# NTT123/vietTTS

Measured on NVIDIA H100. Metric: audio_samples_per_sec, higher is better.
Workload: dtype f32 (bf16x3 split products on wgmma tensor cores, fp32 accumulate/storage)

## Files before the change

### viettts_b200/csrc/hifigan.cu

```cuda
#include "vtts_internal.cuh"

using namespace hgpk;

namespace {

__global__ void repack_ups_kernel(const float* __restrict__ w, float* __restrict__ out, int u, int K, int Cin, int Cout, int a) {
  const size_t total = (size_t)u * 2 * Cin * Cout;
  for (size_t idx = blockIdx.x * (size_t)blockDim.x + threadIdx.x; idx < total; idx += (size_t)gridDim.x * blockDim.x) {
    int o = idx % Cout;
    int i = (idx / Cout) % Cin;
    int q = (idx / ((size_t)Cout * Cin)) % 2;
    int r = idx / ((size_t)Cout * Cin * 2);
    int j0 = ((a - r) % u + u) % u;
    int j = j0 + q * u;
    out[idx] = w[((size_t)j * Cout + o) * Cin + i];
  }
}

__global__ void __launch_bounds__(256) conv_post_kernel(const float* __restrict__ a0, const float* __restrict__ a1,
                                                        const float* __restrict__ a2, const float* __restrict__ w,
                                                        const float* __restrict__ bias, const int* __restrict__ len,
                                                        int len_mul, int R, float* __restrict__ wav) {
  constexpr int C = 32, KW = 7, TT = 256, ST = 33;
  __shared__ float xs[(TT + KW - 1) * ST];
// ... 54 lines not shown

void carve(Arena& ar, int B, int T, HgBufs& hb) {
  const size_t frames = (size_t)B * T;
  hb.P0 = ar.take<float>(frames * 512);
  const size_t big = frames * 8192;
  for (int p = 0; p < 2; ++p)
    for (int j = 0; j < 3; ++j) hb.A[p][j] = ar.take<float>(big);
  hb.X = ar.take<float>(big);
  for (int j = 0; j < 3; ++j) hb.Tb[j] = ar.take<float>(big);
  for (int j = 0; j < 3; ++j) hb.Bb[j] = ar.take<float>(big);
}

}

size_t vtts_hifigan_ws_bytes(int B, int T) {
  Arena ar(nullptr, 0, true);
  HgBufs hb;
  carve(ar, B, T, hb);
  return ar.off + 256;
}

int vtts_hifigan_prepare(vtts_ctx* ctx) {
  ModelWeights& m = ctx->hg;
  std::vector<size_t> dn;
  for (int i = 0, C = vc::HG_C0; i < 4; ++i, C /= 2) dn.push_back((size_t)vc::hg_rate(i) * 2 * C * (C / 2));
  int rc = vtts_alloc_tensors(ctx, dn, &m.derived, m.d);
  if (rc) return rc;
  std::vector<PackSpec> pk(2 * PK_COUNT);
  for (int i = 0, C = vc::HG_C0; i < 4; ++i, C /= 2) {
    const int u = vc::hg_rate(i), K = vc::hg_upk(i);
    repack_ups_kernel<<<256, 256>>>(m.t[hgi::UPS_W(i)], m.d[i], u, K, C, C / 2, (K + u - 2 + 1) / 2);
    VTTS_CUDA(cudaGetLastError());
    for (int r = 0; r < u; ++r) pk[PK_UPS(i, r)] = {m.d[i] + (size_t)r * 2 * C * (C / 2), 2, C, C / 2};
  }
  for (int n = 0; n < 12; ++n)
    for (int which = 0; which < 2; ++which)
      for (int j = 0; j < 3; ++j) {
        const int ch = 256 >> (n / 3);
        pk[PK_RB(n, which, j)] = {m.t[hgi::RB_W(n, which, j)], vc::hg_rbk(n % 3), ch, ch};
      }
  pk[PK_PRE] = {m.t[hgi::PRE_W], 7, vc::MEL, vc::HG_C0};
  for (int e = 0; e < PK_COUNT; ++e) {
    pk[PK_COUNT + e] = pk[e];
    pk[PK_COUNT + e].f16 = true;
  }
  VTTS_CUDA(cudaDeviceSynchronize());
  rc = vtts_pack_convs(ctx, m, pk);
  if (rc) return rc;
  VTTS_CUDA(cudaDeviceSynchronize());
  return VTTS_OK;
}


namespace {

int hg_scale(int i) {
// ... 28 lines not shown
}

int hg_ups(vtts_ctx* ctx, int i, const float* const* x, float* out, const int32_t* n_frames, int B, int T, cudaStream_t st) {
  const ModelWeights& M = ctx->hg;
  auto& W = M.t;
  const bool tc = ctx->precision != VTTS_PRECISION_FP32;
  const int f16 = ctx->precision == VTTS_PRECISION_FP16;
  const int pk = f16 ? PK_COUNT : 0;
  const int C = vc::HG_C0 >> i, scale_in = hg_scale(i), rows_in = T * scale_in;
  const int u = vc::hg_rate(i), K = vc::hg_upk(i), Co = C / 2;
  const int a = (K + u - 2 + 1) / 2;
  ConvLaunch L;
  memset(&L, 0, sizeof(L));
  L.B = B; L.len = n_frames; L.len_mul = scale_in;
  L.nprob = u; L.Cin = C; L.Cout = Co;
  L.T_rows = rows_in; L.rows_out = rows_in * u;
  L.pre_mode = (i == 0) ? 1 : 2; L.pre_slope = 0.1f; L.post_act = 0;
  for (int r = 0; r < u; ++r) {
    int j0 = ((a - r) % u + u) % u;
    int e = (r + j0 - a) / u;
    ConvProb p;
    memset(&p, 0, sizeof(p));
    if (i == 0) { p.x0 = x[0]; } else { p.x0 = x[0]; p.x1 = x[1]; p.x2 = x[2]; }
    p.w = M.d[i] + (size_t)r * 2 * C * Co;
    p.bias = W[hgi::UPS_B(i)];
    p.out = out;
    p.k = 2; p.dil = 1; p.in_off = e; p.out_stride = u; p.out_off = r;
    L.p[r] = p;
  }
  if (!tc) return vtts_launch_conv(ctx, L, st);
  const int nph = Co == 256 ? 1 : (Co == 128 ? 4 : 2);
  TcLaunch TL;
  memset(&TL, 0, sizeof(TL));
  TL.nprob = u / nph; TL.nphase = nph; TL.Cin = C; TL.N = Co; TL.in_ld = C; TL.out_ld = Co;
  TL.B = B; TL.T_rows = rows_in; TL.rows_out = rows_in * u; TL.len = n_frames; TL.len_mul = scale_in;
  TL.pre_mode = L.pre_mode; TL.pre_slope = 0.1f; TL.f16 = f16;
  for (int g = 0; g < u / nph; ++g) {
    const ConvProb& c0 = L.p[g * nph];
    TcProb q;
    memset(&q, 0, sizeof(q));
    q.x0 = c0.x0; q.x1 = c0.x1; q.x2 = c0.x2; q.bias = c0.bias; q.out = c0.out;
    q.k = 2; q.dil = 1; q.out_stride = u;
    q.wpk = M.tiles(pk + PK_UPS(i, g * nph))[0]; q.in_off = c0.in_off; q.out_off = g * nph;
    for (int ph = 0; ph < nph; ++ph) {
      const int r = g * nph + ph;
      q.wpk_ph[ph] = M.tiles(pk + PK_UPS(i, r))[0];
      q.in_off_ph[ph] = L.p[r].in_off;
      q.out_off_ph[ph] = r;
    }
    TL.p[g] = q;
  }
  return vtts_launch_tc_conv(ctx, TL, st);
}

int hg_resblock(vtts_ctx* ctx, int i, int m, const float* const* src, float* const* dst, float* const* tmp, const int32_t* n_frames,
                int B, int T, cudaStream_t st) {
  const ModelWeights& M = ctx->hg;
  auto& W = M.t;
  const bool tc = ctx->precision != VTTS_PRECISION_FP32;
  const int f16 = ctx->precision == VTTS_PRECISION_FP16;
  const int pk = f16 ? PK_COUNT : 0;
  const int Co = vc::HG_C0 >> (i + 1), scale = hg_scale(i + 1), rows = T * scale;
  const int d = vc::hg_dil(m);
  if (tc && ctx->fuse_pairs && Co <= 64) {
    TcPairLaunch PL;
    memset(&PL, 0, sizeof(PL));
    PL.nprob = 3; PL.N = Co; PL.B = B; PL.T_rows = rows; PL.len = n_frames; PL.len_mul = scale; PL.slope = 0.1f; PL.f16 = f16;
    for (int j = 0; j < 3; ++j) {
      const int kk = vc::hg_rbk(j), n = i * 3 + j;
      PL.p[j] = TcPairProb{src[j], M.tiles(pk + PK_RB(n, 0, m))[0], M.tiles(pk + PK_RB(n, 1, m))[0], W[hgi::RB_B(n, 0, m)], W[hgi::RB_B(n, 1, m)],
                           dst[j], kk, d};
    }
    return vtts_launch_tc_pair(ctx, PL, st);
// ... 146 lines not shown
```

### viettts_b200/csrc/tc_conv.cu

```cuda
#include <cuda_bf16.h>

#include <algorithm>

#include "tc_common.cuh"
#include "vtts_internal.cuh"

namespace {

using namespace tcx;

constexpr int NCWG = 2;
constexpr int NCONS = NCWG * 128;
constexpr int PROD_WARP = NCONS / 32;
constexpr int NCONV = 96;
constexpr int NTHREADS = NCONS + 32 + NCONV;
constexpr int NA = 4;
constexpr int HALO = 64;
constexpr int PAIR_OVERLAP = 16;
constexpr int NQ = 2;
constexpr int NREADERS = (NCONS + NCONV) / 32;

template <int N, int MW, int PAIRF, bool STAGED = false>
struct TcCfg {
  static constexpr int R = 64 * MW * NCWG;
  static constexpr int R_OUT = R - PAIR_OVERLAP;
  static constexpr int RA = R + HALO;
  static constexpr int A_STAGE = RA * 64;
  static constexpr int W_STAGE = N * 64;
  static constexpr int NW = N == 256 ? 4 : 8;
  static constexpr int NCH2 = PAIRF ? N / 16 : 0;
  static constexpr int EPI_NC = N < 128 ? N : 128;
  static constexpr int EPI_LD = EPI_NC + 8;
  static constexpr int EPI_WG = 64 * EPI_LD + N;
  static constexpr int EPI_STAGE = STAGED ? NCWG * EPI_WG * 4 : 0;
  static constexpr int SMEM_BYTES =
      NA * A_STAGE + NW * W_STAGE + NCH2 * A_STAGE + EPI_STAGE + (2 * NA + 2 * NW + 2 * NQ) * 8 + NQ * 4 + 1024;
  static_assert(SMEM_BYTES <= 227 * 1024, "shared memory of one CTA");
};

struct Ring {
  uint32_t s = 0, p = 0;
  template <int NS>
  __device__ __forceinline__ void next() { if (++s == NS) { s = 0; p ^= 1; } }
};

struct Tile {
  int pi, b, tt, ph;
};
__device__ __forceinline__ Tile decode_tile(int t, int nph, int nprob, int tiles_per_row) {
  Tile d;
  d.ph = t % nph; t /= nph;
  d.pi = t % nprob; t /= nprob;
  d.tt = t % tiles_per_row;
  d.b = t / tiles_per_row;
  return d;
}

__device__ __forceinline__ int take_ticket(int* sched, int ntiles) {
  const int t = (int)gridDim.x + atomicAdd(&sched[0], 1);
  if (t < ntiles) return t;
  __threadfence();
  if (atomicAdd(&sched[1], 1) == (int)gridDim.x - 1) {
    atomicExch(&sched[0], 0);
    atomicExch(&sched[1], 0);
  }
  return -1;
}

struct TileQueue {
  int* id;
  uint64_t* full;
  uint64_t* empty;
  Ring r;
  __device__ __forceinline__ void put(int t, int* err, long long& acc) {
// ... 160 lines not shown
  asm volatile("cp.async.cg.shared.global [%0], [%1], 16;" ::"r"(smem_u32(smem_dst)), "l"(gsrc) : "memory");
}
__device__ __forceinline__ void cp_async_commit() { asm volatile("cp.async.commit_group;" ::: "memory"); }
__device__ __forceinline__ void cp_async_wait_all() { asm volatile("cp.async.wait_all;" ::: "memory"); }

__device__ __forceinline__ void init_barriers(uint64_t* bars, int nw) {
  uint64_t* a_full = bars;
  uint64_t* a_empty = bars + NA;
  uint64_t* w_full = bars + 2 * NA;
  uint64_t* w_empty = bars + 2 * NA + nw;
  uint64_t* q_full = bars + 2 * NA + 2 * nw;
  uint64_t* q_empty = q_full + NQ;
  for (int i = 0; i < NA; ++i) { mbar_init(&a_full[i], NCONV); mbar_init(&a_empty[i], NCONS / 32); }
  for (int i = 0; i < nw; ++i) { mbar_init(&w_full[i], 1); mbar_init(&w_empty[i], NCONS / 32); }
  for (int i = 0; i < NQ; ++i) { mbar_init(&q_full[i], 1); mbar_init(&q_empty[i], NREADERS); }
  asm volatile("fence.mbarrier_init.release.cluster;" ::: "memory");
}

__device__ __forceinline__ TileQueue tile_queue(uint64_t* bars, int nw) {
  uint64_t* q_full = bars + 2 * NA + 2 * nw;
  return TileQueue{reinterpret_cast<int*>(q_full + 2 * NQ), q_full, q_full + NQ, Ring{}};
}

#define PRODUCER_TILES                                                                     \
  TileQueue q = tile_queue(bars, NW);                                                      \
  long long w_q = 0;                                                                       \
  int t_next = blockIdx.x;                                                                 \
  q.put(t_next, L.err, w_q);                                                               \
  auto next_tile = [&]() {                                                                 \
    const int t = t_next;                                                                  \
    if (t >= 0) { t_next = take_ticket(L.sched, L.ntiles); q.put(t_next, L.err, w_q); }    \
    return t;                                                                              \
  };
#define READER_TILES                                                                       \
  TileQueue q = tile_queue(bars, NW);                                                      \
  long long w_q = 0;                                                                       \
  auto next_tile = [&]() { return q.get(L.err, w_q); };

template <int N, int EPI, int MW, bool F16>
__global__ void __launch_bounds__(NTHREADS, 1) tc_conv_kernel(const __grid_constant__ TcLaunch L) {
  using Cfg = TcCfg<N, MW, 0, EPI == 0>;
  constexpr int R = Cfg::R, RA = Cfg::RA, NW = Cfg::NW;
  extern __shared__ uint8_t smem_raw[];
  uint8_t* smem = (uint8_t*)(((uintptr_t)smem_raw + 1023) & ~(uintptr_t)1023);
  uint8_t* a_st = smem;
  uint8_t* w_st = smem + NA * Cfg::A_STAGE;
  float* epi_st = reinterpret_cast<float*>(smem_raw + (w_st + NW * Cfg::W_STAGE - smem_raw));
  uint64_t* bars = reinterpret_cast<uint64_t*>(w_st + NW * Cfg::W_STAGE + Cfg::EPI_STAGE);
  uint64_t* a_full = bars;
  uint64_t* a_empty = bars + NA;
  uint64_t* w_full = bars + 2 * NA;
  uint64_t* w_empty = bars + 2 * NA + NW;

  const int tid = threadIdx.x;
  const int warp = __shfl_sync(0xffffffffu, tid >> 5, 0);
  if (tid == 0) init_barriers(bars, NW);
  __syncthreads();

  const int nch = L.Cin / 16;
  const int nph = L.nphase > 1 ? L.nphase : 1;

  constexpr bool ROW_BOUNDS = EPI == 0;
#define TILE_LOOP_BEGIN                                                           \
  for (int tile; (tile = next_tile()) >= 0;) {                                    \
    const Tile td = decode_tile(tile, nph, L.nprob, L.tiles_per_row);              \
    const int ph = td.ph, b = td.b;                                                 \
    const int tau0 = td.tt * R;                                                    \
    const TcProb& P = L.p[td.pi];                                                  \
    int valid = L.T_rows, in_lo = 0, out_hi = 0;                                  \
    if (ROW_BOUNDS && P.rb) {                                                     \
      in_lo = P.rb[3 * b]; valid = P.rb[3 * b + 1]; out_hi = P.rb[3 * b + 2];     \
      if (tau0 * P.out_stride + P.out_off_ph[ph] >= out_hi) continue;             \
    } else {                                                                      \
      if (L.len) {                                                                \
        const int v = L.len[b] * L.len_mul;                                       \
        valid = v < valid ? v : valid;                                            \
      }                                                                           \
      if (tau0 >= valid) continue;                                                \
    }
#define TILE_LOOP_END }

  if (warp == PROD_WARP) {
    if ((tid & 31) == 0) {
      Ring rw;
      long long w_e = 0;
      PRODUCER_TILES
      TILE_LOOP_BEGIN
        (void)b; (void)tau0; (void)in_lo; (void)valid; (void)out_hi;
        produce_weights<N, NW, F16>(w_st, w_full, w_empty, rw, P.wpk_ph[ph], nch, P.k, L.err, w_e);
      TILE_LOOP_END
      if (L.dbg) L.dbg[(size_t)blockIdx.x * 16 + 4] = w_e;
    }
  } else if (warp > PROD_WARP) {
    const int ct = tid - NCONS - 32;
    Ring ra;
    long long w_ae = 0;
    READER_TILES
    TILE_LOOP_BEGIN
      const int k = P.k, dil = P.dil;
      const size_t in_base = (size_t)b * L.T_rows * L.in_ld;
      const float* x1 = L.pre_mode == 2 ? P.x1 + in_base : nullptr;
      const float* x2 = L.pre_mode == 2 ? P.x2 + in_base : nullptr;
      for (int c = 0; c < nch; ++c) {
        mbar_wait_t(&a_empty[ra.s], ra.p ^ 1, L.err, 5, w_ae);
        convert_chunk<RA, F16>(a_st + ra.s * Cfg::A_STAGE, ct, P.x0 + in_base, x1, x2, L.in_ld, c, tau0 + P.in_off_ph[ph], R + (k - 1) * dil,
                          in_lo, valid, L.pre_mode, L.pre_slope);
        fence_proxy_async();
        mbar_arrive(&a_full[ra.s]);
        ra.next<NA>();
      }
      (void)out_hi;
    TILE_LOOP_END
    if (L.dbg && ct == 0) L.dbg[(size_t)blockIdx.x * 16 + 5] = w_ae;
  } else {
    const int wg = warp >> 2, lane = tid & 31;
    float acc[MW][N / 2];
    Ring ra, rw;
    long long w_a = 0, w_w = 0, t_epi = 0;
    const long long t_begin = clock64();
    const int n_valid = (EPI && L.n_valid > 0) ? L.n_valid : N;
    const int post_act = EPI ? L.post_act : 0;
    constexpr int EPI_NC = Cfg::EPI_NC, EPI_LD = Cfg::EPI_LD, RPS = 128 / (EPI_NC / 4), NQ4 = 64 / RPS;
    float* stg = epi_st + wg * Cfg::EPI_WG;
    float* stg_bias = stg + 64 * EPI_LD;
    const int fr = (warp & 3) * 16 + (lane >> 2), fc = 2 * (lane & 3);
    const int dr = (tid & 127) / (EPI_NC / 4), dq = (tid & 127) % (EPI_NC / 4);
    READER_TILES
    TILE_LOOP_BEGIN
      const size_t out_base = (size_t)b * L.rows_out * L.out_ld;
      const int ostride = P.out_stride, ooff = P.out_off_ph[ph];
      auto row_ok = [&](int tau) { return (ROW_BOUNDS && P.rb) ? tau * ostride + ooff < out_hi : tau < valid; };
      auto fetch_pass = [&](int mt, int nh) {
        if (P.resid) {
          const int blk = tau0 + (wg * MW + mt) * 64;
#pragma unroll
          for (int i = 0; i < NQ4; ++i) {
            const int row = i * RPS + dr, tau = blk + row;
            if (row_ok(tau))
              cp_async16(stg + row * EPI_LD + dq * 4, P.resid + out_base + ((tau * ostride + ooff) * L.out_ld + nh * EPI_NC + dq * 4));
          }
        }
        cp_async_commit();
      };
      auto wait_pass = [&]() {
        cp_async_wait_all();
        named_bar(2 + wg, 128);
      };
      if constexpr (EPI == 0) {
        if ((tid & 127) < N / 4) cp_async16(stg_bias + (tid & 127) * 4, P.bias + (tid & 127) * 4);
        fetch_pass(0, 0);
      }
      consume<N, MW, RA, NW, true, false, F16>(acc, wg, smem_u32(a_st), a_full, a_empty, ra, smem_u32(w_st), w_full, w_empty, rw, nch, P.k,
                                               P.dil, L.err, w_a, w_w);
      const long long t_epi0 = clock64();
      if constexpr (EPI == 0) {
        wait_pass();
#pragma unroll
        for (int mt = 0; mt < MW; ++mt) {
          if (!row_ok(tau0 + (wg * MW + mt) * 64)) break;
#pragma unroll
          for (int nh = 0; nh < N / EPI_NC; ++nh) {
            if (mt + nh > 0 && P.resid) {
              fetch_pass(mt, nh);
              wait_pass();
            }
#pragma unroll
            for (int jn = 0; jn < EPI_NC / 8; ++jn) {
              const int col = jn * 8 + fc, e = (nh * (EPI_NC / 8) + jn) * 4;
              const float2 bi = *reinterpret_cast<const float2*>(stg_bias + nh * EPI_NC + col);
#pragma unroll
              for (int h = 0; h < 2; ++h) {
                float2* s = reinterpret_cast<float2*>(stg + (fr + 8 * h) * EPI_LD + col);
                float2 o = make_float2(acc[mt][e + 2 * h] + bi.x, acc[mt][e + 2 * h + 1] + bi.y);
                if (P.resid) {
                  const float2 r = *s;
                  o.x += r.x; o.y += r.y;
                }
                *s = o;
              }
            }
            named_bar(2 + wg, 128);
            const int blk = tau0 + (wg * MW + mt) * 64;
#pragma unroll
            for (int i = 0; i < NQ4; ++i) {
              const int row = i * RPS + dr, tau = blk + row;
              if (row_ok(tau))
                *reinterpret_cast<float4*>(P.out + out_base + ((tau * ostride + ooff) * L.out_ld + nh * EPI_NC + dq * 4)) =
                    *reinterpret_cast<const float4*>(stg + row * EPI_LD + dq * 4);
            }
            named_bar(2 + wg, 128);
          }
        }
      } else {
        const int row_w = tau0 + wg * MW * 64 + (warp & 3) * 16 + (lane >> 2);
#pragma unroll
        for (int mt = 0; mt < MW; ++mt)
#pragma unroll
          for (int h = 0; h < 2; ++h) {
            const int tau = row_w + mt * 64 + 8 * h;
            if (!row_ok(tau)) continue;
            const size_t orow = out_base + (size_t)(tau * ostride + ooff) * L.out_ld;
#pragma unroll
            for (int jn = 0; jn < N / 8; ++jn) {
              const int col = jn * 8 + 2 * (lane & 3);
              if (col >= n_valid) continue;
              float2 o = make_float2(acc[mt][jn * 4 + 2 * h], acc[mt][jn * 4 + 2 * h + 1]);
              const float2 bi = __ldg(reinterpret_cast<const float2*>(P.bias + col));
              o.x += bi.x; o.y += bi.y;
              if (P.bn_mean) {
                const float2 mu = __ldg(reinterpret_cast<const float2*>(P.bn_mean + col));
                const float2 iv = __ldg(reinterpret_cast<const float2*>(P.bn_inv + col));
// ... 23 lines not shown

template <int N, int MW, bool A2_REGS, bool F16>
__global__ void __launch_bounds__(NTHREADS, 1) tc_pair_kernel(const __grid_constant__ TcPairLaunch L) {
  using Cfg = TcCfg<N, MW, 1>;
  constexpr int R = Cfg::R, R_OUT = Cfg::R_OUT, RA = Cfg::RA, NW = Cfg::NW, NCH = N / 16;
  extern __shared__ uint8_t smem_raw[];
  uint8_t* smem = (uint8_t*)(((uintptr_t)smem_raw + 1023) & ~(uintptr_t)1023);
  uint8_t* a_st = smem;
  uint8_t* w_st = smem + NA * Cfg::A_STAGE;
  uint8_t* mid = w_st + NW * Cfg::W_STAGE;
  uint64_t* bars = reinterpret_cast<uint64_t*>(mid + Cfg::NCH2 * Cfg::A_STAGE);
  uint64_t* a_full = bars;
  uint64_t* a_empty = bars + NA;
  uint64_t* w_full = bars + 2 * NA;
  uint64_t* w_empty = bars + 2 * NA + NW;

  const int tid = threadIdx.x;
  const int warp = __shfl_sync(0xffffffffu, tid >> 5, 0);
  if (tid == 0) init_barriers(bars, NW);
  __syncthreads();

#define TILE_LOOP_BEGIN                                                   \
  for (int tile; (tile = next_tile()) >= 0;) {                            \
    const Tile td = decode_tile(tile, 1, L.nprob, L.tiles_per_row);        \
    const int b = td.b;                                                    \
    const int tau0 = td.tt * R_OUT;                                        \
    int valid = L.T_rows;                                                 \
    if (L.len) {                                                          \
      const int v = L.len[b] * L.len_mul;                                 \
      valid = v < valid ? v : valid;                                      \
    }                                                                     \
    if (tau0 >= valid) continue;                                          \
    const TcPairProb& P = L.p[td.pi];                                      \
    const int k = P.k, dil = P.dil, h2 = (k - 1) / 2;
#define TILE_LOOP_END }

  if (warp == PROD_WARP) {
    if ((tid & 31) == 0) {
      Ring rw;
      long long w_e = 0;
      PRODUCER_TILES
      TILE_LOOP_BEGIN
        (void)b; (void)tau0; (void)dil; (void)h2;
        produce_weights<N, NW, F16>(w_st, w_full, w_empty, rw, P.w1pk, NCH, k, L.err, w_e);
        produce_weights<N, NW, F16>(w_st, w_full, w_empty, rw, P.w2pk, NCH, k, L.err, w_e);
      TILE_LOOP_END
    }
// ... 86 lines not shown

template <bool F16>
__global__ void pack_w_kernel(const float* __restrict__ w, uint16_t* __restrict__ dst, int k, int Cin, int Cout_total, int n0, int N) {
  const size_t total = (size_t)k * Cin * N;
  for (size_t idx = blockIdx.x * (size_t)blockDim.x + threadIdx.x; idx < total; idx += (size_t)gridDim.x * blockDim.x) {
    const int n = idx % N;
    const int i = (idx / N) % Cin;
    const int j = idx / ((size_t)N * Cin);
    const float v = (n0 + n) < Cout_total ? w[((size_t)j * Cin + i) * Cout_total + n0 + n] : 0.f;
    const int c = i / 16, kh = (i % 16) / 8, e = i % 8;
    if constexpr (F16) {
      const size_t blk = ((size_t)c * k + j) * (size_t)(2 * N * 8);
      dst[blk + ((size_t)kh * N + n) * 8 + e] = (uint16_t)(f16x2_sat(v, 0.f) & 0xffffu);
      continue;
    }
    const __nv_bfloat16 hi = __float2bfloat16_rn(v);
    const __nv_bfloat16 lo = __float2bfloat16_rn(v - __bfloat162float(hi));
    const size_t blk = ((size_t)c * k + j) * (size_t)(4 * N * 8);
    dst[blk + ((size_t)(kh * 2 + 0) * N + n) * 8 + e] = __bfloat16_as_ushort(hi);
    dst[blk + ((size_t)(kh * 2 + 1) * N + n) * 8 + e] = __bfloat16_as_ushort(lo);
  }
}

template <int N, int EPI, int MW, bool F16>
int launch_cfg(vtts_ctx* ctx, TcLaunch& L, cudaStream_t st) {
  using Cfg = TcCfg<N, MW, 0, EPI == 0>;
  static bool attr_done_dev[64] = {};
  if (!attr_done_dev[ctx->device & 63]) {
    VTTS_CUDA(cudaFuncSetAttribute(tc_conv_kernel<N, EPI, MW, F16>, cudaFuncAttributeMaxDynamicSharedMemorySize, Cfg::SMEM_BYTES));
    attr_done_dev[ctx->device & 63] = true;
  }
  const int nph = L.nphase > 1 ? L.nphase : 1;
  for (int i = 0; i < L.nprob; ++i) {
    if (nph == 1) {
      L.p[i].wpk_ph[0] = L.p[i].wpk;
      L.p[i].in_off_ph[0] = L.p[i].in_off;
      L.p[i].out_off_ph[0] = L.p[i].out_off;
    }
    if ((L.p[i].k - 1) * L.p[i].dil > HALO) return ctx->fail(VTTS_ERR_BAD_ARG, "tc_conv: halo too large");
  }
  std::stable_sort(L.p, L.p + L.nprob, [](const TcProb& a, const TcProb& b) { return a.k > b.k; });
  L.tiles_per_row = ((L.tile_rows > 0 ? L.tile_rows : L.T_rows) + Cfg::R - 1) / Cfg::R;
  L.ntiles = L.nprob * L.tiles_per_row * L.B * nph;
  const int grid = L.ntiles < ctx->sm_count ? L.ntiles : ctx->sm_count;
  tc_conv_kernel<N, EPI, MW, F16><<<grid, NTHREADS, Cfg::SMEM_BYTES, st>>>(L);
  ctx->launches++;
  VTTS_CUDA(cudaGetLastError());
  return VTTS_OK;
}

template <int N>
int launch_n(vtts_ctx* ctx, TcLaunch& L, cudaStream_t st) {
  constexpr int MW = N >= 256 ? 1 : (N == 128 ? 2 : 4);
  bool generic = L.post_act != 0 || (L.n_valid > 0 && L.n_valid < N);
  bool rb = false;
  for (int i = 0; i < L.nprob; ++i) {
    generic |= L.p[i].bn_mean != nullptr;
    rb |= L.p[i].rb != nullptr;
  }
  if (rb && generic) return ctx->fail(VTTS_ERR_BAD_ARG, "tc_conv: per-row bounds use the plain epilogue");
  if (!generic) {
    if ((int64_t)L.rows_out * L.out_ld > INT32_MAX) return ctx->fail(VTTS_ERR_BAD_ARG, "tc_conv: %d output rows of %d", L.rows_out, L.out_ld);
    bool aligned = L.out_ld % 4 == 0;
    for (int i = 0; i < L.nprob; ++i) aligned &= (((uintptr_t)L.p[i].out | (uintptr_t)L.p[i].resid | (uintptr_t)L.p[i].bias) & 15) == 0;
    if (!aligned) return ctx->fail(VTTS_ERR_BAD_ARG, "tc_conv: the plain epilogue needs 16-byte aligned out / resid rows and bias (out_ld %d)", L.out_ld);
  }
  if (L.nphase > 4) return ctx->fail(VTTS_ERR_BAD_ARG, "tc_conv: %d phases", L.nphase);
  if (L.nphase > 1 && generic) return ctx->fail(VTTS_ERR_BAD_ARG, "tc_conv: multi-phase tiles use the plain epilogue");
  if (L.f16 && generic) return ctx->fail(VTTS_ERR_BAD_ARG, "tc_conv: fp16 operands use the plain epilogue");
  if (L.f16) return launch_cfg<N, 0, MW, true>(ctx, L, st);
  return generic ? launch_cfg<N, 1, MW, false>(ctx, L, st) : launch_cfg<N, 0, MW, false>(ctx, L, st);
}

template <int N, int MW, bool A2_REGS, bool F16 = false>
int launch_pair(vtts_ctx* ctx, TcPairLaunch& L, cudaStream_t st) {
  using Cfg = TcCfg<N, MW, 1>;
  static bool attr_done_dev[64] = {};
  if (!attr_done_dev[ctx->device & 63]) {
    VTTS_CUDA(cudaFuncSetAttribute(tc_pair_kernel<N, MW, A2_REGS, F16>, cudaFuncAttributeMaxDynamicSharedMemorySize, Cfg::SMEM_BYTES));
    attr_done_dev[ctx->device & 63] = true;
  }
  for (int i = 0; i < L.nprob; ++i)
    if (L.p[i].k - 1 > PAIR_OVERLAP || (L.p[i].k - 1) * L.p[i].dil > HALO) return ctx->fail(VTTS_ERR_BAD_ARG, "tc_pair: halo too large");
  std::stable_sort(L.p, L.p + L.nprob, [](const TcPairProb& a, const TcPairProb& b) { return a.k > b.k; });
  L.tiles_per_row = (L.T_rows + Cfg::R_OUT - 1) / Cfg::R_OUT;
  L.ntiles = L.nprob * L.tiles_per_row * L.B;
  const int grid = L.ntiles < ctx->sm_count ? L.ntiles : ctx->sm_count;
  tc_pair_kernel<N, MW, A2_REGS, F16><<<grid, NTHREADS, Cfg::SMEM_BYTES, st>>>(L);
  ctx->launches++;
  VTTS_CUDA(cudaGetLastError());
  return VTTS_OK;
}

}
// ... 109 lines not shown
```

### viettts_b200/csrc/vocoder_stream.cu

```cuda
#include <algorithm>

#include "stream_common.cuh"

using namespace hgpk;

namespace {

constexpr int NRATE = 5;
constexpr int NTEN = 2 + 4 * 19;
constexpr int NCONV = 1 + 4 * 19;

struct Plan {
  int rate[NRATE];
  int lead[NRATE];
  int lag_p0;
  int lag_in[4];
  int late[4];
  int lag_x[4];
  int lag_t[4][3][3], lag_y[4][3][3];
  int lag_m[4];
  int D;
};

constexpr int ups_e(int i, int r) {
// ... 193 lines not shown
  if (ctx->precision == VTTS_PRECISION_FP32)
    return ctx->fail(VTTS_ERR_BAD_ARG, "vocoder_stream_push: the strict fp32 mode has no streaming path; use bf16x3 or fp16");
  const int S = vs->S, F = vs->F;
  const Plan& pl = plan();
  const int D = pl.D, wav_ld = vc::HOP * (F + D);
  SlotState& sl = vs->slots;
  rc = sl.check(ctx, "vocoder_stream_push", F, n_new, flags);
  if (rc) return rc;
  VTTS_CUDA(cudaSetDevice(ctx->device));
  cudaStream_t st = (cudaStream_t)stream;

  std::vector<int> P0(S), act(S), end(S), nn(S);
  for (int s = 0; s < S; ++s) {
    act[s] = n_new[s] > 0 || flags[s] != 0;
    end[s] = (flags[s] & 2) != 0;
    nn[s] = n_new[s];
    P0[s] = (flags[s] & 1) ? 0 : (int)sl.P[s];
  }
  const size_t o_post = (size_t)NCONV * S * 3, o_prep = o_post + (size_t)S * 4, n_tbl = o_prep + (size_t)S * 3;
  vs->tbl.assign(n_tbl, 0);
  int* tb = vs->tbl.data();
  int tile_rows[NCONV];
  std::fill(tile_rows, tile_rows + NCONV, 1);
  auto bounds = [&](int c, int ri_in, int lag_in, int ri_out, int lag_out, int u) {
    const int sin = pl.rate[ri_in], sout = pl.rate[ri_out];
    const int out0 = u > 1 ? pl.lead[ri_out] - lag_out + pl.late[ri_in] - u : pl.lead[ri_out] - lag_out;
    for (int s = 0; s < S; ++s) {
      if (!act[s]) continue;
      int* r = tb + ((size_t)c * S + s) * 3;
      r[0] = std::max(0, pl.lead[ri_in] - sin * P0[s]);
      r[1] = sin * nn[s] + pl.lead[ri_in] - (end[s] ? 0 : lag_in);
      r[2] = sout * nn[s] + pl.lead[ri_out] - (end[s] ? 0 : lag_out);
      tile_rows[c] = std::max(tile_rows[c], (r[2] - out0 + u - 1) / u);
    }
  };
  bounds(0, 0, 0, 0, pl.lag_p0, 1);
  for (int i = 0; i < 4; ++i) {
    bounds(ci_ups(i), i, pl.lag_in[i], i + 1, pl.lag_x[i], vc::hg_rate(i));
    for (int m = 0; m < 3; ++m)
      for (int j = 0; j < 3; ++j) {
        bounds(ci_rb(i, m, 0, j), i + 1, m == 0 ? pl.lag_x[i] : pl.lag_y[i][j][m - 1], i + 1, pl.lag_t[i][j][m], 1);
        bounds(ci_rb(i, m, 1, j), i + 1, pl.lag_t[i][j][m], i + 1, pl.lag_y[i][j][m], 1);
      }
  }
  std::vector<int> emit(S, 0), P1(S);
  std::vector<long long> E1(S);
  int post_max = 0;
  for (int s = 0; s < S; ++s) {
    P1[s] = P0[s] + nn[s];
// ... 23 lines not shown
  stream_prep_kernel<<<dim3(NTEN, S), 256, 0, st>>>(vs->d_ten, dtb + o_prep, mel_dev, F);
  ctx->launches++;
  VTTS_CUDA(cudaGetLastError());

  const ModelWeights& M = ctx->hg;
  auto& W = M.t;
  const int f16 = ctx->precision == VTTS_PRECISION_FP16;
  const int pk = f16 ? PK_COUNT : 0;
  auto rb = [&](int c) { return dtb + (size_t)c * S * 3; };
  const auto& T = vs->ten;
  TcLaunch TL;
  memset(&TL, 0, sizeof(TL));
  TL.nprob = 2; TL.Cin = vc::MEL; TL.N = 256; TL.in_ld = vc::MEL; TL.out_ld = vc::HG_C0;
  TL.B = S; TL.T_rows = vs->cap[0]; TL.rows_out = vs->cap[0]; TL.tile_rows = tile_rows[0]; TL.pre_mode = 0; TL.pre_slope = 1.f; TL.f16 = f16;
  for (int t = 0; t < 2; ++t) {
    TcProb& q = TL.p[t];
    q.x0 = T[0].p; q.wpk = M.tiles(pk + PK_PRE)[t]; q.bias = W[hgi::PRE_B] + 256 * t; q.out = T[1].p + 256 * t;
    q.k = 7; q.dil = 1; q.in_off = pl.lead[0] - pl.lag_p0 - 3; q.out_stride = 1; q.out_off = pl.lead[0] - pl.lag_p0; q.rb = rb(0);
  }
  if ((rc = vtts_launch_tc_conv(ctx, TL, st))) return rc;

  for (int i = 0, C = vc::HG_C0; i < 4; ++i, C /= 2) {
    const int u = vc::hg_rate(i), Co = C / 2;
    const int nph = Co == 256 ? 1 : (Co == 128 ? 4 : 2);
    memset(&TL, 0, sizeof(TL));
    TL.nprob = u / nph; TL.nphase = nph; TL.Cin = C; TL.N = Co; TL.in_ld = C; TL.out_ld = Co;
    TL.B = S; TL.T_rows = vs->cap[i]; TL.rows_out = vs->cap[i + 1]; TL.tile_rows = tile_rows[ci_ups(i)];
    TL.pre_mode = i == 0 ? 1 : 2; TL.pre_slope = 0.1f; TL.f16 = f16;
    for (int g = 0; g < u / nph; ++g) {
      TcProb& q = TL.p[g];
      if (i == 0) {
        q.x0 = T[1].p;
      } else {
        q.x0 = T[ti_y(i - 1, 0, 2)].p; q.x1 = T[ti_y(i - 1, 1, 2)].p; q.x2 = T[ti_y(i - 1, 2, 2)].p;
      }
      q.bias = W[hgi::UPS_B(i)]; q.out = T[ti_x(i)].p; q.k = 2; q.dil = 1; q.out_stride = u; q.rb = rb(ci_ups(i));
      for (int ph = 0; ph < nph; ++ph) {
        const int r = g * nph + ph;
        q.wpk_ph[ph] = M.tiles(pk + PK_UPS(i, r))[0];
        q.in_off_ph[ph] = pl.lead[i] - pl.lag_in[i] - 1 + ups_e(i, r);
        q.out_off_ph[ph] = pl.lead[i + 1] - pl.lag_x[i] + pl.late[i] - u + r;
      }
      q.wpk = q.wpk_ph[0]; q.in_off = q.in_off_ph[0]; q.out_off = q.out_off_ph[0];
    }
    if ((rc = vtts_launch_tc_conv(ctx, TL, st))) return rc;

    for (int m = 0; m < 3; ++m) {
      const int d = vc::hg_dil(m);
      for (int which = 0; which < 2; ++which) {
        const int c0 = ci_rb(i, m, which, 0);
        memset(&TL, 0, sizeof(TL));
        TL.nprob = 3; TL.Cin = Co; TL.N = Co; TL.in_ld = Co; TL.out_ld = Co;
        TL.B = S; TL.T_rows = vs->cap[i + 1]; TL.rows_out = vs->cap[i + 1];
        TL.pre_mode = 1; TL.pre_slope = 0.1f; TL.f16 = f16;
        for (int j = 0; j < 3; ++j) {
          const int kk = vc::hg_rbk(j), n = i * 3 + j, c = c0 + j;
          const int dd = which == 0 ? d : 1, h = (kk - 1) * dd / 2;
          const int lag_out = which == 0 ? pl.lag_t[i][j][m] : pl.lag_y[i][j][m];
          const float* x = m == 0 ? T[ti_x(i)].p : T[ti_y(i, j, m - 1)].p;
          TcProb& q = TL.p[j];
          q.x0 = which == 0 ? x : T[ti_t(i, j, m)].p;
          q.wpk = M.tiles(pk + PK_RB(n, which, m))[0];
          q.bias = W[hgi::RB_B(n, which, m)];
          q.resid = which == 0 ? nullptr : x;
          q.out = which == 0 ? T[ti_t(i, j, m)].p : T[ti_y(i, j, m)].p;
          q.k = kk; q.dil = dd; q.in_off = pl.lead[i + 1] - lag_out - h; q.out_stride = 1; q.out_off = pl.lead[i + 1] - lag_out;
// ... 31 lines not shown
```

### viettts_b200/csrc/vtts_internal.cuh

```cuda
#pragma once
#include <cuda_runtime.h>
#include <stdint.h>
#include <stdio.h>
#include <string.h>
#include <algorithm>
#include <string>
#include <vector>

#include "../../include/viettts_b200.h"

namespace vc {
constexpr int MEL = 80;
constexpr int HOP = 256;
constexpr int NFFT = 1024;
constexpr int NBINS = 513;
constexpr int ENC_D = 256;
constexpr int ENC_OUT = 512;
constexpr int DEC_H = 512;
constexpr int PRENET = 256;
constexpr int POSTNET = 512;
constexpr int VOCAB = 256;
constexpr int SIL_INDEX = 0;
constexpr int WORD_END_INDEX = 3;
constexpr int HG_C0 = 512;
// ... 34 lines not shown
  int Cin, Cout;
  int B;
  int T_rows;
  int rows_out;
  const int* len;
  int len_mul;
  int pre_mode;
  float pre_slope;
  int post_act;
};

struct TcProb {
  const float* x0;
  const float* x1;
  const float* x2;
  const void* wpk;
  const float* bias;
  const float* resid;
  const float* bn_mean;
  const float* bn_inv;
  const float* bn_off;
  float* out;
  int k, dil, in_off, out_stride, out_off;
  const void* wpk_ph[4];
  int in_off_ph[4];
  int out_off_ph[4];
  const int* rb;
};

struct TcLaunch {
  TcProb p[8];
  int nprob;
  int Cin, N;
  int in_ld, out_ld;
  int B, T_rows, rows_out;
  const int* len;
  int len_mul;
  int pre_mode;
  float pre_slope;
  int nphase;
  int post_act;
  int n_valid;
  int f16;
  int tile_rows;
  int tiles_per_row, ntiles;
  int* sched;
  int* err;
  long long* dbg;
};

struct TcPairProb {
  const float* x;
  const void* w1pk;
  const void* w2pk;
  const float* b1;
  const float* b2;
  float* out;
  int k, dil;
};

struct TcPairLaunch {
  TcPairProb p[3];
  int nprob;
// ... 222 lines not shown
int vtts_denoise_ola(vtts_ctx* ctx, const float* x, long long x_ld, int S, const int* n_in, const DnRow* rows, int B, long long max_out,
                     const float* ws, int ws_frames, float* y, long long y_ld, cudaStream_t st);
int vtts_fft_tables(vtts_ctx* ctx);
int vtts_melspec_prepare(vtts_ctx* ctx);
int vtts_melspec_run(vtts_ctx* ctx, const float* wav, int B, int S, float* mel, cudaStream_t st);

struct TensorSpec { const char* name; int64_t n; };
const std::vector<TensorSpec>& vtts_hifigan_specs();
const std::vector<TensorSpec>& vtts_acoustic_specs();
const std::vector<TensorSpec>& vtts_duration_specs();

namespace hgi {
constexpr int PRE_W = 0, PRE_B = 1;
__host__ __device__ constexpr int UPS_W(int i) { return 2 + 2 * i; }
__host__ __device__ constexpr int UPS_B(int i) { return 3 + 2 * i; }
__host__ __device__ constexpr int RB_W(int n, int which, int m) { return 10 + n * 12 + (which * 3 + m) * 2; }
__host__ __device__ constexpr int RB_B(int n, int which, int m) { return RB_W(n, which, m) + 1; }
constexpr int POST_W = 10 + 12 * 12, POST_B = POST_W + 1;
constexpr int COUNT = POST_B + 1;
}

namespace hgpk {
constexpr int PK_RB(int n, int which, int m) { return n * 6 + which * 3 + m; }
constexpr int PK_UPS(int i, int r) { return i == 0 ? 72 + r : PK_UPS(i - 1, vc::hg_rate(i - 1)) + r; }
constexpr int PK_PRE = PK_UPS(4, 0), PK_COUNT = PK_PRE + 1;
}

namespace aci {
constexpr int EMBED = 0;
__host__ __device__ constexpr int ENC_CONV(int i, int f) { return 1 + i * 6 + f; }
constexpr int ENC_LSTM_F_W = 19, ENC_LSTM_F_B = 20, ENC_LSTM_B_W = 21, ENC_LSTM_B_B = 22;
constexpr int DEC_L0_W = 23, DEC_L0_B = 24, DEC_L1_W = 25, DEC_L1_B = 26;
constexpr int PROJ_W = 27, PROJ_B = 28, PRE1_W = 29, PRE2_W = 30;
__host__ __device__ constexpr int POST_CONV(int i, int f) { return 31 + i * 6 + f; }
constexpr int COUNT = 31 + 4 * 6 + 2;
}

namespace dui {
constexpr int FC1_W = 23, FC1_B = 24, FC2_W = 25, FC2_B = 26;
constexpr int COUNT = 27;
}
```

Measured before the change: 53.35 million.

## Fuse upsample phases into one wide GEMM with sub-row interleaved output

Replaces the per-phase transposed-conv decomposition, where each of the u output phases was a separate tile or phase of a k=2 conv, with a single GEMM whose N dimension concatenates all u phases' weights (u*Co columns). The phases are reordered so that they share a common input offset. The output is written contiguously as sub-rows through a new SUB epilogue mode with per-element bounds. This widens N for the small-channel stages, improving tensor-core tile utilisation, and removes the per-phase weight and input re-streaming. It adds element-level bounds checks and a new kernel template variant.

```diff
diff --git a/viettts_b200/csrc/hifigan.cu b/viettts_b200/csrc/hifigan.cu
--- a/viettts_b200/csrc/hifigan.cu
+++ b/viettts_b200/csrc/hifigan.cu
@@ -100,16 +100,25 @@
 
 int vtts_hifigan_prepare(vtts_ctx* ctx) {
   ModelWeights& m = ctx->hg;
-  std::vector<size_t> dn;
-  for (int i = 0, C = vc::HG_C0; i < 4; ++i, C /= 2) dn.push_back((size_t)vc::hg_rate(i) * 2 * C * (C / 2));
+  std::vector<size_t> dn(12);
+  for (int i = 0, C = vc::HG_C0; i < 4; ++i, C /= 2) {
+    dn[D_UPS_PH(i)] = dn[D_UPS_BLK(i)] = (size_t)vc::hg_rate(i) * 2 * C * (C / 2);
+    dn[D_UPS_BLK_B(i)] = (size_t)vc::hg_rate(i) * (C / 2);
+  }
   int rc = vtts_alloc_tensors(ctx, dn, &m.derived, m.d);
   if (rc) return rc;
   std::vector<PackSpec> pk(2 * PK_COUNT);
   for (int i = 0, C = vc::HG_C0; i < 4; ++i, C /= 2) {
-    const int u = vc::hg_rate(i), K = vc::hg_upk(i);
-    repack_ups_kernel<<<256, 256>>>(m.t[hgi::UPS_W(i)], m.d[i], u, K, C, C / 2, (K + u - 2 + 1) / 2);
+    const int u = vc::hg_rate(i), K = vc::hg_upk(i), Co = C / 2;
+    repack_ups_kernel<<<256, 256>>>(m.t[hgi::UPS_W(i)], m.d[D_UPS_PH(i)], u, K, C, Co, (K + u - 2 + 1) / 2);
     VTTS_CUDA(cudaGetLastError());
-    for (int r = 0; r < u; ++r) pk[PK_UPS(i, r)] = {m.d[i] + (size_t)r * 2 * C * (C / 2), 2, C, C / 2};
+    for (int mm = 0; mm < u; ++mm) {
+      const int r = (mm + u / 2) % u;
+      VTTS_CUDA(cudaMemcpy2D(m.d[D_UPS_BLK(i)] + (size_t)mm * Co, (size_t)u * Co * 4, m.d[D_UPS_PH(i)] + (size_t)r * 2 * C * Co, (size_t)Co * 4,
+                             (size_t)Co * 4, 2 * C, cudaMemcpyDeviceToDevice));
+      VTTS_CUDA(cudaMemcpy(m.d[D_UPS_BLK_B(i)] + (size_t)mm * Co, m.t[hgi::UPS_B(i)], (size_t)Co * 4, cudaMemcpyDeviceToDevice));
+    }
+    pk[PK_UPS(i)] = {m.d[D_UPS_BLK(i)], 2, C, u * Co};
   }
   for (int n = 0; n < 12; ++n)
     for (int which = 0; which < 2; ++which)
@@ -184,33 +193,24 @@
     ConvProb p;
     memset(&p, 0, sizeof(p));
     if (i == 0) { p.x0 = x[0]; } else { p.x0 = x[0]; p.x1 = x[1]; p.x2 = x[2]; }
-    p.w = M.d[i] + (size_t)r * 2 * C * Co;
+    p.w = M.d[D_UPS_PH(i)] + (size_t)r * 2 * C * Co;
     p.bias = W[hgi::UPS_B(i)];
     p.out = out;
     p.k = 2; p.dil = 1; p.in_off = e; p.out_stride = u; p.out_off = r;
     L.p[r] = p;
   }
   if (!tc) return vtts_launch_conv(ctx, L, st);
-  const int nph = Co == 256 ? 1 : (Co == 128 ? 4 : 2);
+  const int N = vtts_tc_tile_n(u * Co), nt = u * Co / N;
   TcLaunch TL;
   memset(&TL, 0, sizeof(TL));
-  TL.nprob = u / nph; TL.nphase = nph; TL.Cin = C; TL.N = Co; TL.in_ld = C; TL.out_ld = Co;
-  TL.B = B; TL.T_rows = rows_in; TL.rows_out = rows_in * u; TL.len = n_frames; TL.len_mul = scale_in;
+  TL.nprob = nt; TL.Cin = C; TL.N = N; TL.in_ld = C; TL.out_ld = u * Co; TL.out_sub = Co;
+  TL.B = B; TL.T_rows = rows_in; TL.rows_out = rows_in * u; TL.tile_rows = rows_in + 1; TL.len = n_frames; TL.len_mul = scale_in;
   TL.pre_mode = L.pre_mode; TL.pre_slope = 0.1f; TL.f16 = f16;
-  for (int g = 0; g < u / nph; ++g) {
-    const ConvProb& c0 = L.p[g * nph];
-    TcProb q;
-    memset(&q, 0, sizeof(q));
-    q.x0 = c0.x0; q.x1 = c0.x1; q.x2 = c0.x2; q.bias = c0.bias; q.out = c0.out;
-    q.k = 2; q.dil = 1; q.out_stride = u;
-    q.wpk = M.tiles(pk + PK_UPS(i, g * nph))[0]; q.in_off = c0.in_off; q.out_off = g * nph;
-    for (int ph = 0; ph < nph; ++ph) {
-      const int r = g * nph + ph;
-      q.wpk_ph[ph] = M.tiles(pk + PK_UPS(i, r))[0];
-      q.in_off_ph[ph] = L.p[r].in_off;
-      q.out_off_ph[ph] = r;
-    }
-    TL.p[g] = q;
+  for (int g = 0; g < nt; ++g) {
+    TcProb& q = TL.p[g];
+    q.x0 = L.p[0].x0; q.x1 = L.p[0].x1; q.x2 = L.p[0].x2;
+    q.wpk = M.tiles(pk + PK_UPS(i))[g]; q.bias = M.d[D_UPS_BLK_B(i)] + g * N; q.out = out;
+    q.k = 2; q.dil = 1; q.in_off = -1; q.out_stride = 1; q.out_off = 0; q.out_e0 = -(u / 2) * Co + g * N;
   }
   return vtts_launch_tc_conv(ctx, TL, st);
 }
diff --git a/viettts_b200/csrc/tc_conv.cu b/viettts_b200/csrc/tc_conv.cu
--- a/viettts_b200/csrc/tc_conv.cu
+++ b/viettts_b200/csrc/tc_conv.cu
@@ -45,11 +45,10 @@
 };
 
 struct Tile {
-  int pi, b, tt, ph;
+  int pi, b, tt;
 };
-__device__ __forceinline__ Tile decode_tile(int t, int nph, int nprob, int tiles_per_row) {
+__device__ __forceinline__ Tile decode_tile(int t, int nprob, int tiles_per_row) {
   Tile d;
-  d.ph = t % nph; t /= nph;
   d.pi = t % nprob; t /= nprob;
   d.tt = t % tiles_per_row;
   d.b = t / tiles_per_row;
@@ -256,6 +255,10 @@
   return TileQueue{reinterpret_cast<int*>(q_full + 2 * NQ), q_full, q_full + NQ, Ring{}};
 }
 
+__device__ __forceinline__ int sub_elem(const TcLaunch& L, const TcProb& P, int tau, int col) {
+  return (tau * P.out_stride + P.out_off) * L.out_ld + P.out_e0 + col;
+}
+
 #define PRODUCER_TILES                                                                     \
   TileQueue q = tile_queue(bars, NW);                                                      \
   long long w_q = 0;                                                                       \
@@ -271,8 +274,9 @@
   long long w_q = 0;                                                                       \
   auto next_tile = [&]() { return q.get(L.err, w_q); };
 
-template <int N, int EPI, int MW, bool F16>
+template <int N, int EPI, int MW, bool F16, bool SUB>
 __global__ void __launch_bounds__(NTHREADS, 1) tc_conv_kernel(const __grid_constant__ TcLaunch L) {
+  static_assert(!SUB || EPI == 0, "sub-row output uses the plain epilogue");
   using Cfg = TcCfg<N, MW, 0, EPI == 0>;
   constexpr int R = Cfg::R, RA = Cfg::RA, NW = Cfg::NW;
   extern __shared__ uint8_t smem_raw[];
@@ -292,26 +296,27 @@
   __syncthreads();
 
   const int nch = L.Cin / 16;
-  const int nph = L.nphase > 1 ? L.nphase : 1;
 
   constexpr bool ROW_BOUNDS = EPI == 0;
 #define TILE_LOOP_BEGIN                                                           \
   for (int tile; (tile = next_tile()) >= 0;) {                                    \
-    const Tile td = decode_tile(tile, nph, L.nprob, L.tiles_per_row);              \
-    const int ph = td.ph, b = td.b;                                                 \
+    const Tile td = decode_tile(tile, L.nprob, L.tiles_per_row);                   \
+    const int b = td.b;                                                            \
     const int tau0 = td.tt * R;                                                    \
     const TcProb& P = L.p[td.pi];                                                  \
     int valid = L.T_rows, in_lo = 0, out_hi = 0;                                  \
     if (ROW_BOUNDS && P.rb) {                                                     \
       in_lo = P.rb[3 * b]; valid = P.rb[3 * b + 1]; out_hi = P.rb[3 * b + 2];     \
-      if (tau0 * P.out_stride + P.out_off_ph[ph] >= out_hi) continue;             \
+      if (!SUB && tau0 * P.out_stride + P.out_off >= out_hi) continue;            \
     } else {                                                                      \
       if (L.len) {                                                                \
         const int v = L.len[b] * L.len_mul;                                       \
         valid = v < valid ? v : valid;                                            \
       }                                                                           \
-      if (tau0 >= valid) continue;                                                \
-    }
+      if (!SUB && tau0 >= valid) continue;                                        \
+    }                                                                             \
+    const int e_lim = SUB ? (P.rb ? out_hi * L.out_sub : valid * L.out_ld) : 0;   \
+    if (SUB && sub_elem(L, P, tau0, 0) >= e_lim) continue;
 #define TILE_LOOP_END }
 
   if (warp == PROD_WARP) {
@@ -320,8 +325,8 @@
       long long w_e = 0;
       PRODUCER_TILES
       TILE_LOOP_BEGIN
-        (void)b; (void)tau0; (void)in_lo; (void)valid; (void)out_hi;
-        produce_weights<N, NW, F16>(w_st, w_full, w_empty, rw, P.wpk_ph[ph], nch, P.k, L.err, w_e);
+        (void)b; (void)tau0; (void)in_lo; (void)valid; (void)out_hi; (void)e_lim;
+        produce_weights<N, NW, F16>(w_st, w_full, w_empty, rw, P.wpk, nch, P.k, L.err, w_e);
       TILE_LOOP_END
       if (L.dbg) L.dbg[(size_t)blockIdx.x * 16 + 4] = w_e;
     }
@@ -337,13 +342,13 @@
       const float* x2 = L.pre_mode == 2 ? P.x2 + in_base : nullptr;
       for (int c = 0; c < nch; ++c) {
         mbar_wait_t(&a_empty[ra.s], ra.p ^ 1, L.err, 5, w_ae);
-        convert_chunk<RA, F16>(a_st + ra.s * Cfg::A_STAGE, ct, P.x0 + in_base, x1, x2, L.in_ld, c, tau0 + P.in_off_ph[ph], R + (k - 1) * dil,
+        convert_chunk<RA, F16>(a_st + ra.s * Cfg::A_STAGE, ct, P.x0 + in_base, x1, x2, L.in_ld, c, tau0 + P.in_off, R + (k - 1) * dil,
                           in_lo, valid, L.pre_mode, L.pre_slope);
         fence_proxy_async();
         mbar_arrive(&a_full[ra.s]);
         ra.next<NA>();
       }
-      (void)out_hi;
+      (void)out_hi; (void)e_lim;
     TILE_LOOP_END
     if (L.dbg && ct == 0) L.dbg[(size_t)blockIdx.x * 16 + 5] = w_ae;
   } else {
@@ -361,17 +366,18 @@
     const int dr = (tid & 127) / (EPI_NC / 4), dq = (tid & 127) % (EPI_NC / 4);
     READER_TILES
     TILE_LOOP_BEGIN
-      const size_t out_base = (size_t)b * L.rows_out * L.out_ld;
-      const int ostride = P.out_stride, ooff = P.out_off_ph[ph];
+      const size_t out_base = (size_t)b * L.rows_out * (SUB ? L.out_sub : L.out_ld);
+      const int ostride = P.out_stride, ooff = P.out_off, oe0 = SUB ? P.out_e0 : 0;
       auto row_ok = [&](int tau) { return (ROW_BOUNDS && P.rb) ? tau * ostride + ooff < out_hi : tau < valid; };
+      auto elem_ok = [&](int tau, int e) { return SUB ? e >= 0 && e < e_lim : row_ok(tau); };
       auto fetch_pass = [&](int mt, int nh) {
         if (P.resid) {
           const int blk = tau0 + (wg * MW + mt) * 64;
 #pragma unroll
           for (int i = 0; i < NQ4; ++i) {
             const int row = i * RPS + dr, tau = blk + row;
-            if (row_ok(tau))
-              cp_async16(stg + row * EPI_LD + dq * 4, P.resid + out_base + ((tau * ostride + ooff) * L.out_ld + nh * EPI_NC + dq * 4));
+            const int e = (tau * ostride + ooff) * L.out_ld + oe0 + nh * EPI_NC + dq * 4;
+            if (elem_ok(tau, e)) cp_async16(stg + row * EPI_LD + dq * 4, P.resid + out_base + e);
           }
         }
         cp_async_commit();
@@ -391,7 +397,8 @@
         wait_pass();
 #pragma unroll
         for (int mt = 0; mt < MW; ++mt) {
-          if (!row_ok(tau0 + (wg * MW + mt) * 64)) break;
+          const int blk = tau0 + (wg * MW + mt) * 64;
+          if (SUB ? sub_elem(L, P, blk, 0) >= e_lim : !row_ok(blk)) break;
 #pragma unroll
           for (int nh = 0; nh < N / EPI_NC; ++nh) {
             if (mt + nh > 0 && P.resid) {
@@ -414,13 +421,12 @@
               }
             }
             named_bar(2 + wg, 128);
-            const int blk = tau0 + (wg * MW + mt) * 64;
 #pragma unroll
             for (int i = 0; i < NQ4; ++i) {
               const int row = i * RPS + dr, tau = blk + row;
-              if (row_ok(tau))
-                *reinterpret_cast<float4*>(P.out + out_base + ((tau * ostride + ooff) * L.out_ld + nh * EPI_NC + dq * 4)) =
-                    *reinterpret_cast<const float4*>(stg + row * EPI_LD + dq * 4);
+              const int e = (tau * ostride + ooff) * L.out_ld + oe0 + nh * EPI_NC + dq * 4;
+              if (elem_ok(tau, e))
+                *reinterpret_cast<float4*>(P.out + out_base + e) = *reinterpret_cast<const float4*>(stg + row * EPI_LD + dq * 4);
             }
             named_bar(2 + wg, 128);
           }
@@ -490,7 +496,7 @@
 
 #define TILE_LOOP_BEGIN                                                   \
   for (int tile; (tile = next_tile()) >= 0;) {                            \
-    const Tile td = decode_tile(tile, 1, L.nprob, L.tiles_per_row);        \
+    const Tile td = decode_tile(tile, L.nprob, L.tiles_per_row);        \
     const int b = td.b;                                                    \
     const int tau0 = td.tt * R_OUT;                                        \
     int valid = L.T_rows;                                                 \
@@ -623,28 +629,21 @@
   }
 }
 
-template <int N, int EPI, int MW, bool F16>
+template <int N, int EPI, int MW, bool F16, bool SUB = false>
 int launch_cfg(vtts_ctx* ctx, TcLaunch& L, cudaStream_t st) {
   using Cfg = TcCfg<N, MW, 0, EPI == 0>;
   static bool attr_done_dev[64] = {};
   if (!attr_done_dev[ctx->device & 63]) {
-    VTTS_CUDA(cudaFuncSetAttribute(tc_conv_kernel<N, EPI, MW, F16>, cudaFuncAttributeMaxDynamicSharedMemorySize, Cfg::SMEM_BYTES));
+    VTTS_CUDA(cudaFuncSetAttribute(tc_conv_kernel<N, EPI, MW, F16, SUB>, cudaFuncAttributeMaxDynamicSharedMemorySize, Cfg::SMEM_BYTES));
     attr_done_dev[ctx->device & 63] = true;
   }
-  const int nph = L.nphase > 1 ? L.nphase : 1;
-  for (int i = 0; i < L.nprob; ++i) {
-    if (nph == 1) {
-      L.p[i].wpk_ph[0] = L.p[i].wpk;
-      L.p[i].in_off_ph[0] = L.p[i].in_off;
-      L.p[i].out_off_ph[0] = L.p[i].out_off;
-    }
+  for (int i = 0; i < L.nprob; ++i)
     if ((L.p[i].k - 1) * L.p[i].dil > HALO) return ctx->fail(VTTS_ERR_BAD_ARG, "tc_conv: halo too large");
-  }
   std::stable_sort(L.p, L.p + L.nprob, [](const TcProb& a, const TcProb& b) { return a.k > b.k; });
   L.tiles_per_row = ((L.tile_rows > 0 ? L.tile_rows : L.T_rows) + Cfg::R - 1) / Cfg::R;
-  L.ntiles = L.nprob * L.tiles_per_row * L.B * nph;
+  L.ntiles = L.nprob * L.tiles_per_row * L.B;
   const int grid = L.ntiles < ctx->sm_count ? L.ntiles : ctx->sm_count;
-  tc_conv_kernel<N, EPI, MW, F16><<<grid, NTHREADS, Cfg::SMEM_BYTES, st>>>(L);
+  tc_conv_kernel<N, EPI, MW, F16, SUB><<<grid, NTHREADS, Cfg::SMEM_BYTES, st>>>(L);
   ctx->launches++;
   VTTS_CUDA(cudaGetLastError());
   return VTTS_OK;
@@ -659,18 +658,20 @@
     generic |= L.p[i].bn_mean != nullptr;
     rb |= L.p[i].rb != nullptr;
   }
-  if (rb && generic) return ctx->fail(VTTS_ERR_BAD_ARG, "tc_conv: per-row bounds use the plain epilogue");
+  if ((rb || L.out_sub) && generic) return ctx->fail(VTTS_ERR_BAD_ARG, "tc_conv: per-row bounds and sub-row output use the plain epilogue");
+  if (L.out_sub < 0 || (L.out_sub && (L.out_sub % 4 || L.out_ld % L.out_sub)))
+    return ctx->fail(VTTS_ERR_BAD_ARG, "tc_conv: output rows of %d floats in tile rows of %d", L.out_sub, L.out_ld);
   if (!generic) {
-    if ((int64_t)L.rows_out * L.out_ld > INT32_MAX) return ctx->fail(VTTS_ERR_BAD_ARG, "tc_conv: %d output rows of %d", L.rows_out, L.out_ld);
+    const int row_w = L.out_sub ? L.out_sub : L.out_ld;
+    if ((int64_t)L.rows_out * row_w > INT32_MAX) return ctx->fail(VTTS_ERR_BAD_ARG, "tc_conv: %d output rows of %d", L.rows_out, row_w);
     bool aligned = L.out_ld % 4 == 0;
     for (int i = 0; i < L.nprob; ++i) aligned &= (((uintptr_t)L.p[i].out | (uintptr_t)L.p[i].resid | (uintptr_t)L.p[i].bias) & 15) == 0;
     if (!aligned) return ctx->fail(VTTS_ERR_BAD_ARG, "tc_conv: the plain epilogue needs 16-byte aligned out / resid rows and bias (out_ld %d)", L.out_ld);
   }
-  if (L.nphase > 4) return ctx->fail(VTTS_ERR_BAD_ARG, "tc_conv: %d phases", L.nphase);
-  if (L.nphase > 1 && generic) return ctx->fail(VTTS_ERR_BAD_ARG, "tc_conv: multi-phase tiles use the plain epilogue");
   if (L.f16 && generic) return ctx->fail(VTTS_ERR_BAD_ARG, "tc_conv: fp16 operands use the plain epilogue");
-  if (L.f16) return launch_cfg<N, 0, MW, true>(ctx, L, st);
-  return generic ? launch_cfg<N, 1, MW, false>(ctx, L, st) : launch_cfg<N, 0, MW, false>(ctx, L, st);
+  if (L.f16) return L.out_sub ? launch_cfg<N, 0, MW, true, true>(ctx, L, st) : launch_cfg<N, 0, MW, true>(ctx, L, st);
+  if (generic) return launch_cfg<N, 1, MW, false>(ctx, L, st);
+  return L.out_sub ? launch_cfg<N, 0, MW, false, true>(ctx, L, st) : launch_cfg<N, 0, MW, false>(ctx, L, st);
 }
 
 template <int N, int MW, bool A2_REGS, bool F16 = false>
diff --git a/viettts_b200/csrc/vocoder_stream.cu b/viettts_b200/csrc/vocoder_stream.cu
--- a/viettts_b200/csrc/vocoder_stream.cu
+++ b/viettts_b200/csrc/vocoder_stream.cu
@@ -239,9 +239,11 @@
   int* tb = vs->tbl.data();
   int tile_rows[NCONV];
   std::fill(tile_rows, tile_rows + NCONV, 1);
+  auto ups_out0 = [&](int i) { return pl.lead[i + 1] - pl.lag_x[i] + pl.late[i] - vc::hg_rate(i) - vc::hg_rate(i) / 2; };
+  auto ups_in_off = [&](int i) { return pl.lead[i] - pl.lag_in[i] - 2; };
   auto bounds = [&](int c, int ri_in, int lag_in, int ri_out, int lag_out, int u) {
     const int sin = pl.rate[ri_in], sout = pl.rate[ri_out];
-    const int out0 = u > 1 ? pl.lead[ri_out] - lag_out + pl.late[ri_in] - u : pl.lead[ri_out] - lag_out;
+    const int out0 = u > 1 ? ups_out0(ri_in) : pl.lead[ri_out] - lag_out;
     for (int s = 0; s < S; ++s) {
       if (!act[s]) continue;
       int* r = tb + ((size_t)c * S + s) * 3;
@@ -311,26 +313,21 @@
 
   for (int i = 0, C = vc::HG_C0; i < 4; ++i, C /= 2) {
     const int u = vc::hg_rate(i), Co = C / 2;
-    const int nph = Co == 256 ? 1 : (Co == 128 ? 4 : 2);
+    const int N = vtts_tc_tile_n(u * Co), nt = u * Co / N;
     memset(&TL, 0, sizeof(TL));
-    TL.nprob = u / nph; TL.nphase = nph; TL.Cin = C; TL.N = Co; TL.in_ld = C; TL.out_ld = Co;
+    TL.nprob = nt; TL.Cin = C; TL.N = N; TL.in_ld = C; TL.out_ld = u * Co; TL.out_sub = Co;
     TL.B = S; TL.T_rows = vs->cap[i]; TL.rows_out = vs->cap[i + 1]; TL.tile_rows = tile_rows[ci_ups(i)];
     TL.pre_mode = i == 0 ? 1 : 2; TL.pre_slope = 0.1f; TL.f16 = f16;
-    for (int g = 0; g < u / nph; ++g) {
+    for (int g = 0; g < nt; ++g) {
       TcProb& q = TL.p[g];
       if (i == 0) {
         q.x0 = T[1].p;
       } else {
         q.x0 = T[ti_y(i - 1, 0, 2)].p; q.x1 = T[ti_y(i - 1, 1, 2)].p; q.x2 = T[ti_y(i - 1, 2, 2)].p;
       }
-      q.bias = W[hgi::UPS_B(i)]; q.out = T[ti_x(i)].p; q.k = 2; q.dil = 1; q.out_stride = u; q.rb = rb(ci_ups(i));
-      for (int ph = 0; ph < nph; ++ph) {
-        const int r = g * nph + ph;
-        q.wpk_ph[ph] = M.tiles(pk + PK_UPS(i, r))[0];
-        q.in_off_ph[ph] = pl.lead[i] - pl.lag_in[i] - 1 + ups_e(i, r);
-        q.out_off_ph[ph] = pl.lead[i + 1] - pl.lag_x[i] + pl.late[i] - u + r;
-      }
-      q.wpk = q.wpk_ph[0]; q.in_off = q.in_off_ph[0]; q.out_off = q.out_off_ph[0];
+      q.wpk = M.tiles(pk + PK_UPS(i))[g]; q.bias = M.d[D_UPS_BLK_B(i)] + g * N; q.out = T[ti_x(i)].p;
+      q.k = 2; q.dil = 1; q.in_off = ups_in_off(i); q.out_stride = 1; q.out_off = 0; q.out_e0 = ups_out0(i) * Co + g * N;
+      q.rb = rb(ci_ups(i));
     }
     if ((rc = vtts_launch_tc_conv(ctx, TL, st))) return rc;
 
diff --git a/viettts_b200/csrc/vtts_internal.cuh b/viettts_b200/csrc/vtts_internal.cuh
--- a/viettts_b200/csrc/vtts_internal.cuh
+++ b/viettts_b200/csrc/vtts_internal.cuh
@@ -80,9 +80,7 @@
   const float* bn_off;
   float* out;
   int k, dil, in_off, out_stride, out_off;
-  const void* wpk_ph[4];
-  int in_off_ph[4];
-  int out_off_ph[4];
+  int out_e0;
   const int* rb;
 };
 
@@ -96,7 +94,7 @@
   int len_mul;
   int pre_mode;
   float pre_slope;
-  int nphase;
+  int out_sub;
   int post_act;
   int n_valid;
   int f16;
@@ -365,8 +363,11 @@
 
 namespace hgpk {
 constexpr int PK_RB(int n, int which, int m) { return n * 6 + which * 3 + m; }
-constexpr int PK_UPS(int i, int r) { return i == 0 ? 72 + r : PK_UPS(i - 1, vc::hg_rate(i - 1)) + r; }
-constexpr int PK_PRE = PK_UPS(4, 0), PK_COUNT = PK_PRE + 1;
+constexpr int PK_UPS(int i) { return 72 + i; }
+constexpr int PK_PRE = PK_UPS(4), PK_COUNT = PK_PRE + 1;
+constexpr int D_UPS_PH(int i) { return i; }
+constexpr int D_UPS_BLK(int i) { return 4 + i; }
+constexpr int D_UPS_BLK_B(int i) { return 8 + i; }
 }
 
 namespace aci {
```

After: 55.45 million, median of 6. 3.9% higher.
